# Suyashagarw/StreamOptima

Hardware: AMD Instinct MI355X
Metric: encoded Mpixels/sec at 1080p & 4K, 1/2/4/8 GPUs; PSNR delta vs reference (higher is better)
Workload: dtype u8

## Files before the change

### include/streamoptima.h

```cpp
#ifndef STREAMOPTIMA_H
#define STREAMOPTIMA_H

#include <stddef.h>
#include <stdint.h>

#ifdef __cplusplus
extern "C" {
#endif

#define SO_OK 0
#define SO_E_INVALID (-1)
#define SO_E_UNSUPPORTED (-2)
#define SO_MAX_REF 4
#define SO_ABI_VERSION 1

int so_abi_version(void);
const char* so_last_error(void);

int so_me_full_search(const uint8_t* cur, const uint8_t* const* refs, int nref, int H,
                      int W, int bs, int sr, int32_t* out_best, int32_t* out_sub,
                      void* stream);

int so_inter_tq_recon(const uint8_t* cur, const uint8_t* const* refs, int nref, int H,
                      int W, int bs, const int32_t* best, const int32_t* sub, int qp_rd,
// ... 17 lines not shown

#define SO_OPT_RUN_2PASS_FUSED 1
#define SO_OPT_FASTME_SERIAL 2
#define SO_OPT_FASTME_SEGMENT 3
#define SO_OPT_FASTME_WARMUP 4
#define SO_OPT_COUNT_SAD_OPS 5
#define SO_OPT_TEST_LOSE_FLAG 6
#define SO_OPT_RUN_ZERO_SKIP 7
#define SO_OPT_RUN_TALL_TILES 8
int so_set_option(int option, int value);
int so_get_option(int option);

#define SO_P_RUN_TIMEOUT_WORD 32
#define SO_P_RUN_FALLBACK_WORD 64
#define SO_P_RUN_SAD_OPS_WORD 66
#define SO_P_RUN_STALE_WORD 33
#define SO_P_RUN_GAP_WORD 34
#define SO_P_RUN_DIAG_WORD 96
#define SO_P_RUN_DIAG_MAGIC 0x534F0001u
size_t so_p_run_workspace_elems(int H, int W);
int so_p_run_resident_workgroups(int vbs);
int so_p_run_mode_resident_workgroups(int mode, int vbs);
int so_p_run_tile_rows(int H, int W, int conc);
int so_encode_p_run(const uint8_t* const* curs, int nframes, const uint8_t* ref0, int H, int W,
                    int bs, int sr, int qp_rd, const int32_t* qp_row, int vbs, double lam,
                    uint8_t* const* out_split,
                    int16_t* const* out_mv, int16_t* const* out_qtc, int32_t* const* out_tokens,
                    int32_t* const* out_mae_num, uint8_t* const* out_recon, int32_t* const* out_sse,
                    uint32_t* workspace, void* stream);

// ... 180 lines not shown
```

### streamoptima_amd/csrc/so_block.h

```cpp
#pragma once
#include "so_common.h"
#include "so_dct.h"

namespace so {

SO_DEV void wave_sync() {
    __builtin_amdgcn_fence(__ATOMIC_RELEASE, "wavefront");
    __builtin_amdgcn_wave_barrier();
    __builtin_amdgcn_fence(__ATOMIC_ACQUIRE, "wavefront");
}

SO_DEV int scan_index(int n, int i, int j) {
    const int k = i + j;
    const int before = (k < n) ? (k * (k + 1)) / 2 : n * n - ((2 * n - 1 - k) * (2 * n - k)) / 2;
    const int first_i = (k < n) ? 0 : k - n + 1;
    return before + (i - first_i);
}

template <int G>
SO_DEV int group_sum(int v) {
#pragma unroll
    for (int m = G / 2; m >= 1; m >>= 1) v += __shfl_xor(v, m, 64);
    return v;
}
// ... 162 lines not shown
#pragma unroll
    for (int r = 0; r < N; ++r) colp[r * P] = (uint32_t)__builtin_bit_cast(uint64_t, v[r]);
    wave_sync();
#pragma unroll
    for (int c = 0; c < N; ++c) lo[c] = rowp[c];
    wave_sync();
#pragma unroll
    for (int r = 0; r < N; ++r) colp[r * P] = (uint32_t)(__builtin_bit_cast(uint64_t, v[r]) >> 32);
    wave_sync();
#pragma unroll
    for (int c = 0; c < N; ++c)
        v[c] = __builtin_bit_cast(double, ((uint64_t)rowp[c] << 32) | (uint64_t)lo[c]);
    if constexpr (INVERSE) dct::dct3<N>(v, tw); else dct::dct2<N>(v, tw);
#pragma unroll
    for (int c = 0; c < N; ++c) out_row[c] = v[c];
    wave_sync();
}

template <class TWt>
SO_DEV void xform2d_fwd_i_half(double* lds, int l, const int* in_row, double* out_row, const TWt& tw) {
    constexpr int N = 16, PI = N + 1, P = 9;
    const int hl = l >> 3, cl = l & 7;
    double v[N];
    {
        int* const li = reinterpret_cast<int*>(lds);
#pragma unroll
        for (int c = 0; c < N; ++c) li[l * PI + c] = in_row[c];
        wave_sync();
        int x[N];
#pragma unroll
// ... 244 lines not shown
```

### streamoptima_amd/csrc/so_dct.h

```cpp
#pragma once
#include "so_common.h"

namespace so {
namespace dct {

constexpr double kTw16Dct[15] = {
    0x1.fd88da3d12526p-1, 0x1.f6297cff75cb0p-1, 0x1.e9f4156c62ddap-1, 0x1.d906bcf328d46p-1,
    0x1.c38b2f180bdb1p-1, 0x1.a9b66290ea1a3p-1, 0x1.8bc806b151741p-1, 0x1.6a09e667f3bccp-1,
    0x1.44cf325091dd6p-1, 0x1.1c73b39ae68c8p-1, 0x1.e2b5d3806f639p-2, 0x1.87de2a6aea961p-2,
    0x1.294062ed59f04p-2, 0x1.8f8b83c69a60ap-3, 0x1.917a6bc29b424p-4};
constexpr double kTw16Rf[9] = {
    0x1.d906bcf328d46p-1, 0x1.87de2a6aea963p-2, 0.0,
    0x1.6a09e667f3bccp-1, 0x1.6a09e667f3bcdp-1, 0.0,
    0x1.87de2a6aea963p-2, 0x1.d906bcf328d46p-1, 0.0};
constexpr double kSqrt2 = 0x1.6a09e667f3bcdp+0;
constexpr double kHsqt2 = 0x1.6a09e667f3bcdp-1;

struct TW16 {
    SO_DEV double dct(int i) const { return kTw16Dct[i]; }
    SO_DEV double hdct(int i) const { return 0.5 * kTw16Dct[i]; }
    SO_DEV double dct2x(int i) const { return 2 * kTw16Dct[i]; }
    SO_DEV double rf(int i) const { return kTw16Rf[i]; }
    SO_DEV double fct() const { return 0x1.6a09e667f3bcdp-3; }
    SO_DEV double sqrt2() const { return kSqrt2; }
// ... 15 lines not shown
    SO_DEV double hsqt2() const { return kHsqt2; }
};

#define SO_TW_D(i) kTw16Dct[i]
#define SO_TW_H(i) (0.5 * kTw16Dct[i])
static __constant__ double kTw16Tab[45] = {
    SO_TW_D(0), SO_TW_D(1), SO_TW_D(2), SO_TW_D(3), SO_TW_D(4), SO_TW_D(5), SO_TW_D(6), SO_TW_D(7),
    SO_TW_D(8), SO_TW_D(9), SO_TW_D(10), SO_TW_D(11), SO_TW_D(12), SO_TW_D(13), SO_TW_D(14),
    SO_TW_H(0), SO_TW_H(1), SO_TW_H(2), SO_TW_H(3), SO_TW_H(4), SO_TW_H(5), SO_TW_H(6), SO_TW_H(7),
    SO_TW_H(8), SO_TW_H(9), SO_TW_H(10), SO_TW_H(11), SO_TW_H(12), SO_TW_H(13), SO_TW_H(14),
    kTw16Rf[0], kTw16Rf[1], kTw16Rf[2], kTw16Rf[3], kTw16Rf[4], kTw16Rf[5], kTw16Rf[6], kTw16Rf[7], kTw16Rf[8],
    0x1.6a09e667f3bcdp-3, kSqrt2, kSqrt2 * 0.5, kHsqt2, 2 * kTw16Dct[7], 0.0};
#undef SO_TW_D
#undef SO_TW_H
typedef const __attribute__((address_space(4))) double* so_cdp;
struct TW16R {
    so_cdp p;
    SO_DEV double dct(int i) const { return p[i]; }
    SO_DEV double hdct(int i) const { return p[15 + i]; }
    SO_DEV double dct2x(int i) const { return i == 7 ? p[43] : 2 * p[i]; }
    SO_DEV double rf(int i) const { return p[30 + i]; }
    SO_DEV double fct() const { return p[39]; }
    SO_DEV double sqrt2() const { return p[40]; }
    SO_DEV double hsqrt2() const { return p[41]; }
    SO_DEV double hsqt2() const { return p[42]; }
};
SO_DEV TW16R tw16_table() {
    so_cdp q = (so_cdp)kTw16Tab;
    asm volatile("" : "+s"(q));
    return TW16R{q};
}
static __constant__ double kTw8Tab[21] = {
    kTw8Dct[0], kTw8Dct[1], kTw8Dct[2], kTw8Dct[3], kTw8Dct[4], kTw8Dct[5], kTw8Dct[6],
    0.5 * kTw8Dct[0], 0.5 * kTw8Dct[1], 0.5 * kTw8Dct[2], 0.5 * kTw8Dct[3], 0.5 * kTw8Dct[4],
    0.5 * kTw8Dct[5], 0.5 * kTw8Dct[6],
    kTw8Rf[0], kTw8Rf[1], 0x1.0p-2, kSqrt2, kSqrt2 * 0.5, kHsqt2, 2 * kTw8Dct[3]};
struct TW8R {
    so_cdp p;
    SO_DEV double dct(int i) const { return p[i]; }
    SO_DEV double hdct(int i) const { return p[7 + i]; }
    SO_DEV double dct2x(int i) const { return i == 3 ? p[20] : 2 * p[i]; }
    SO_DEV double rf(int i) const { return p[14 + i]; }
    SO_DEV double fct() const { return 0x1.0p-2; }
    SO_DEV double sqrt2() const { return p[17]; }
    SO_DEV double hsqrt2() const { return p[18]; }
    SO_DEV double hsqt2() const { return p[19]; }
};
SO_DEV TW8R tw8_table() {
    so_cdp q = (so_cdp)kTw8Tab;
    asm volatile("" : "+s"(q));
    return TW8R{q};
}

#define SO_PM(a, b, c, d) { a = (c) + (d); b = (c) - (d); }
#define SO_MULPM(a, b, c, d, e, f) { a = (c) * (e) + (d) * (f); b = (c) * (f) - (d) * (e); }

template <int IDO, int L1, class TW>
SO_DEV void radf2(const double* cc, double* ch, const TW& tw) {
#define CC(a, b, c) cc[(a) + IDO * ((b) + L1 * (c))]
#define CH(a, b, c) ch[(a) + IDO * ((b) + 2 * (c))]
#define WA(x, i) tw.rf((i) + (x) * (IDO - 1))
#pragma unroll
    for (int k = 0; k < L1; k++) SO_PM(CH(0, 0, k), CH(IDO - 1, 1, k), CC(0, k, 0), CC(0, k, 1));
    if constexpr ((IDO & 1) == 0) {
#pragma unroll
// ... 392 lines not shown
        c[kc] = tw.dct(k - 1) * t1 - tw.dct(kc - 1) * t2;
    }
    c[4] = (double)x[4] * tw.dct2x(3);
    Rfft<8>::forward(c, tw);
#pragma unroll
    for (int k = 1; k < 7; k += 2) {
        double t = c[k];
        c[k] -= c[k + 1];
        c[k + 1] += t;
    }
}

#undef SO_PM
#undef SO_MULPM

}
}
```

### streamoptima_amd/csrc/so_me.hip

```cpp
#include <stdlib.h>
#include <string.h>

#include <cstring>
#include <map>
#include <mutex>
#include <type_traits>
#include <utility>

#include "so_block.h"
#include "so_common.h"
#include "so_dpp.h"
#include "so_run.h"

namespace so {

SO_DEV uint64_t me_key(uint32_t sad, uint32_t l1, uint32_t ref, uint32_t scan) {
    return ((uint64_t)sad << 32) | ((uint64_t)l1 << 24) | ((uint64_t)ref << 16) | (uint64_t)scan;
}
constexpr uint64_t kNoKey = ~0ull;
constexpr uint32_t kDenseSadOps = 1152u * 256u;
#define SO_OPS_ADD(p, v) do { if (L.count_ops) atomicAdd((p), (v)); } while (0)

SO_DEV void decode_key(uint64_t k, int sr, int32_t* out) {
    if (k == kNoKey) {
// ... 513 lines not shown
extern "C" int so_debug_set_sea_stamps(void* p) {
    return (int)hipMemcpyToSymbol(HIP_SYMBOL(g_sea_stamps), &p, sizeof(p));
}
extern "C" int so_debug_set_run_stamps(void* p) {
    return (int)hipMemcpyToSymbol(HIP_SYMBOL(g_run_stamps), &p, sizeof(p));
}
#else
#define SO_STAMP_REC_SET(p) do { } while (0)
#define SO_SEA_STAMP(i, v) do { } while (0)
#endif

#define SO_MARK_NAMES(X) X(loop_top) X(stage_cur) X(stage_cur_int) X(stage_cur_edge) X(cur_sums) X(wait) \
    X(poll_iter) X(stage_win) X(stage_win_int) X(stage_win_edge) X(dense_tile) X(dense_tile_block) X(byte_sums) \
    X(block_top) X(bound) X(umin) X(umin_edge) X(ballots) X(bal_row) X(dense_fallback) X(survivors) X(sur_one) X(sur_le4) X(sur_pass) \
    X(search_end) X(decode_keys) X(tq_residual) X(tq_fwd) X(tq_quant) X(tq_tokens) X(tq_qtc_store) X(tq_inv) \
    X(tq_recon) X(tq_sse_records) X(post) X(done_flag) X(task_end) X(vbs_block) X(vbs_umin) X(vbs_list_a) \
    X(vbs_pass) X(vbs_list_b) X(vbs_final) X(vbs_dense) X(vbs_fwd) X(vbs_fwd_sub) X(vbs_final_q) X(vbs_inv) \
    X(vbs_inv_split) X(vbs_inv_end) X(wait_w0) X(keys_tail) X(p1_tq) X(p1_flag) X(p2_wait) X(p2_sums) X(p2_tq) \
    X(p2_flag)
#define SO_MARK_ENUM(n) kMark_##n,
enum SoMarkId { SO_MARK_NAMES(SO_MARK_ENUM) kMarkCount };
#undef SO_MARK_ENUM
#if defined(SO_MARKS_COUNT)
__device__ unsigned* g_mark_counts = nullptr;
__shared__ unsigned s_mark_cnt[64];
extern "C" int so_debug_set_mark_counts(void* p) {
    return (int)hipMemcpyToSymbol(HIP_SYMBOL(g_mark_counts), &p, sizeof(p));
}
SO_DEV void so_mark_hit(int id) {
    uint64_t sv, m;
    uint32_t f;
// ... 945 lines not shown
};

struct PHalo {
    uint8_t* up;
    uint8_t* dn;
    int up_end, dn_begin;
};

#ifdef SO_TQ_TW_LITERAL
#define SO_TQ_TW() dct::TW16{}
#define SO_TQ_TW8() dct::TW8{}
#else
#define SO_TQ_TW() dct::tw16_table()
#define SO_TQ_TW8() dct::tw8_table()
#endif
template <class G, bool SC1, bool HALO = false, bool TOK = false, bool HALFTQ = false, bool ZSKIP = false>
SO_DEV void tq16_exact(PTileLds<G, false, HALFTQ>& S, int g, int l, double* scratch, int bx0, int byt0, int nbx, int by0, int by1,
                       int W, int qp_rd, const int32_t* __restrict__ qp_row, const int32_t* __restrict__ qp_map,
                       const PFrameOut& o, const PHalo& hl = PHalo{}, bool qs = false) {
    constexpr int SR = G::SR, TBX = G::TBX;
    const int bxl = g % TBX, byl = g / TBX;
    const int gbx = bx0 + bxl, gby = byt0 + byl;
    if (gbx < nbx && gby < by1) {
        const size_t b = (size_t)(gby - by0) * nbx + gbx;
        const int x = gbx * 16, y = gby * 16;
        const int qpr = qp_map ? qp_map[(size_t)gby * nbx + gbx] : (qp_row ? qp_row[gby] : qp_rd);
        const int dx = S.mer[g][0], dy = S.mer[g][1], rf = S.mer[g][2], sad = S.mer[g][3];
        const int prow = byl * 16 + SR + dy + l, pcol = bxl * 16 + SR + dx;
        const uint32_t* crow = S.curt + (byl * 16 + l) * G::CPD + bxl * 4;
        double* dl = scratch;
        constexpr double kRne = 0x1.8p52;
        int q[16];
        if (qs) {
            const so_v4u* qr = reinterpret_cast<const so_v4u*>(reinterpret_cast<const int16_t*>(dl) + l * 16);
#pragma unroll
            for (int h = 0; h < 2; ++h) {
                const so_v4u v = qr[h];
#pragma unroll
                for (int e = 0; e < 4; ++e) {
                    q[8 * h + 2 * e] = (int)(int16_t)(v[e] & 0xFFFFu);
                    q[8 * h + 2 * e + 1] = (int)v[e] >> 16;
                }
            }
        } else {
            SO_MARK(tq_residual);
            int res[16];
            {
                uint32_t pw[4];
                win_row16<G::RP>(S.win, prow, pcol, pw);
#pragma unroll
                for (int k = 0; k < 4; ++k) {
                    const uint32_t cw = crow[k];
#pragma unroll
                    for (int e = 0; e < 4; ++e)
                        res[4 * k + e] = (int)((cw >> (8 * e)) & 255) - (int)((pw[k] >> (8 * e)) & 255);
                }
            }
            double tcr[16];
            SO_MARK(tq_fwd);
            static_assert(!HALFTQ || TOK, "the half scratch carries the forward transform only");
            if constexpr (HALFTQ)
                xform2d_fwd_i_half(dl, l, res, tcr, SO_TQ_TW());
            else if constexpr (G::TQDW)
                xform2d_rows_dw<false>(dl, l, res, tcr, SO_TQ_TW());
            else
                xform2d_rows<16, false>(dl, l, res, tcr, SO_TQ_TW());
            SO_MARK(tq_quant);
#pragma unroll
            for (int c = 0; c < 16; ++c)
                q[c] = (int)(uint32_t)__builtin_bit_cast(
                    uint64_t, __builtin_amdgcn_ldexp(__builtin_rint(tcr[c]), -q_exp_fast<16>(l, c, qpr)) + kRne);
        }
        SO_MARK(tq_tokens);
        const int tok = block_tokens<16>(nullptr, l, q);
        if constexpr (TOK) {
            if (l == 0) o.tokens[b] = tok;
            return;
        }
        SO_MARK(tq_qtc_store);
        store_row_i16<16>(o.qtc + b * 256 + l * 16, q);
        const auto finish = [&](const int (&rec)[16]) -> int {
            if constexpr (SC1) {
                so_v4u v;
#pragma unroll
                for (int k = 0; k < 4; ++k)
                    v[k] = (uint32_t)(rec[4 * k] & 255) | ((uint32_t)(rec[4 * k + 1] & 255) << 8) |
                           ((uint32_t)(rec[4 * k + 2] & 255) << 16) | ((uint32_t)(rec[4 * k + 3] & 255) << 24);
                uint8_t* rp = o.recon + (size_t)(y + l) * W + x;
// ... 21 lines not shown
                    crow2 = S.curt + ((g2 / TBX) * 16 + l2) * G::CPD + (g2 % TBX) * 4;
                }
#pragma unroll
                for (int k = 0; k < 4; ++k) {
                    const uint32_t cw = crow2[k];
#pragma unroll
                    for (int e = 0; e < 4; ++e) {
                        const int d = (int)((cw >> (8 * e)) & 255) - (rec[4 * k + e] & 255);
                        e2 += d * d;
                    }
                }
                e2 = group_sum<16>(e2);
            }
            return e2;
        };
        const auto full = [&]() -> int {
            int dq[16];
            double rd[16];
            dequant_row_int<16>(q, l, qpr, dq);
            SO_MARK(tq_inv);
            if constexpr (G::TQDW)
                xform2d_rows_dw<true>(dl, l, dq, rd, SO_TQ_TW());
            else
                xform2d_rows<16, true>(dl, l, dq, rd, SO_TQ_TW());
            SO_MARK(tq_recon);
            int rec[16];
            {
                uint32_t pw[4];
                win_row16<G::RP>(S.win, prow, pcol, pw);
#pragma unroll
                for (int c = 0; c < 16; ++c)
                    rec[c] = (int)((pw[c >> 2] >> (8 * (c & 3))) & 255) +
                             (int)(uint32_t)__builtin_bit_cast(uint64_t, rd[c] + kRne);
            }
            return finish(rec);
        };
        int sse;
        if constexpr (ZSKIP) {
            if (__builtin_amdgcn_ballot_w64(tok != 1) == 0) {
                int rec[16];
                uint32_t pw[4];
                win_row16<G::RP>(S.win, prow, pcol, pw);
#pragma unroll
                for (int c = 0; c < 16; ++c) rec[c] = (int)((pw[c >> 2] >> (8 * (c & 3))) & 255);
                sse = finish(rec);
            } else {
                sse = full();
            }
        } else {
            sse = full();
// ... 419 lines not shown
    SO_MARK(vbs_inv_end);
    if (o.sse) {
        sse = group_sum<16>(sse);
        if (l == 0) o.sse[b] = sse;
    }
}

SO_DEV void store_sc1_i16(int16_t* p, int v) {
    asm volatile("global_store_short %0, %1, off sc1" ::"v"(p), "v"(v) : "memory");
}
SO_DEV void store_sc1_i32(int32_t* p, int v) {
    asm volatile("global_store_dword %0, %1, off sc1" ::"v"(p), "v"(v) : "memory");
}

template <class G, bool SC1, class Pre = NoPre, bool HALO = false, bool TOK = false, bool VBS = false,
          class Post = NoPre, bool HALFTQ = false, bool ZSKIP = false, int LISTS = 0>
SO_DEV void ptile_body(PTileLds<G, VBS, HALFTQ>& S, int tile, const uint8_t* __restrict__ cur, const uint8_t* ref, int H, int W,
                       int by0, int by1, int qp_rd, const int32_t* __restrict__ qp_row,
                       const int32_t* __restrict__ qp_map, int32_t* __restrict__ out_best, const PFrameOut& o,
                       const Pre& pre = Pre(), const PHalo& hl = PHalo{}, double lam = 0.0,
                       const int* dense_flag = nullptr, int32_t* fb_out = nullptr, int count_ops = 0,
                       const Post& post = Post(), const int16_t* prev_mv = nullptr) {
    constexpr int SR = G::SR, TBX = G::TBX, TBY = G::TBY;
    using P = PTileGeo<G>;
    uint32_t* const b4w = reinterpret_cast<uint32_t*>(S.un);
    uint16_t* const list = reinterpret_cast<uint16_t*>(b4w + P::B4);
    constexpr int kUnDw = 2 * (VBS ? PTileGeoVbs<G>::U64 : PTileGeo<G, HALFTQ>::U64);
    int dense4 = 0;
#ifndef SO_DENSE_ONE
    if constexpr (3 * G::DCS + 32 <= kUnDw) {
        const int d = (int)((reinterpret_cast<uintptr_t>(b4w) - reinterpret_cast<uintptr_t>(S.win)) / 4);
// ... 54 lines not shown
        }
        if (SO_PROF_PHASE == 1 && ln < 16 * G::TQ_BPW && gq < G::NBLK) {
            const int bxl = gq % G::TBX, byl = gq / G::TBX, l = ln & 15;
            const int gbx = bx0 + bxl, gby = byt0 + byl;
            if (gbx < nbx && gby < by1) {
                const uint32_t* crow = S.curt + (byl * 16 + l) * G::CPD + bxl * 4;
                so_v4u v;
                for (int k = 0; k < 4; ++k) v[k] = crow[k];
                *reinterpret_cast<so_v4u*>(o.recon + (size_t)(gby * 16 + l) * W + gbx * 16) = v;
            }
        } else if (ln < 16 * G::TQ_BPW && gq < G::NBLK) {
            if constexpr (VBS)
                tq16_vbs_fwd<G, SC1, HALO>(S, gq, ln & 15, S.un + gq * kTqScratchVbs, bx0, byt0, nbx, by0, by1, W, qp_rd,
                                           qp_row, qp_map, lam, o);
            else
                tq16_exact<G, SC1, HALO, TOK, HALFTQ, ZSKIP>(S, gq, ln & 15, S.un + gq * tq_scratch<G, HALFTQ>(), bx0,
                                              byt0, nbx, by0, by1, W, qp_rd,
                                              qp_row, qp_map, o, hl, qs);
        }
    }
    if constexpr (VBS) {
        if (SO_PROF_PHASE != 1) {
            __syncthreads();
            const int ln = tid & 63, gq = (tid >> 6) * G::TQ_BPW + (ln >> 4);
            if (ln < 16 * G::TQ_BPW && gq < G::NBLK)
                tq16_vbs_inv<G, SC1, HALO>(S, gq, ln & 15, S.un, bx0, byt0, nbx, by0, by1, W, qp_rd,
                                           qp_row, qp_map, o, hl);
        }
    }
    SO_SEA_STAMP(7, __builtin_amdgcn_s_memtime());
    SO_MARK(post);
// ... 198 lines not shown

#ifndef SO_RUN_ACQUIRE
#define SO_RUN_ACQUIRE 1
#endif
#ifndef SO_RUN_ABORT_CHECK
#define SO_RUN_ABORT_CHECK 1
#endif
#ifndef SO_RUN_TIMEOUT_WORD
#define SO_RUN_TIMEOUT_WORD 32
#endif
#ifndef SO_RUN_DONE_BASE
#define SO_RUN_DONE_BASE 128
#endif
constexpr int kRunTimeoutWord = SO_RUN_TIMEOUT_WORD, kRunDoneBase = SO_RUN_DONE_BASE;
constexpr int kRunExitWord = 1, kRunEpochWord = 2, kRunFallbackWord = 64, kRunSadOpsWord = SO_P_RUN_SAD_OPS_WORD;
constexpr int kRunStaleWord = SO_P_RUN_STALE_WORD, kRunGapWord = SO_P_RUN_GAP_WORD, kRunClaimWord = 35;
constexpr int kRunDiagWord = SO_P_RUN_DIAG_WORD;
static_assert(kRunDoneBase >= kRunDiagWord + 32, "the diagnostic record precedes the done flags");
constexpr int kRunSingle = 0, kRunStripe = 1, kRunFPipe = 2, kRunTwoPass = 3, kRunFPipe2P = 4;
#ifdef SO_RUN_PROFILE
#define SO_RUN_PROF(word, cyc) \
    do { if (wave == 0) __hip_atomic_fetch_add(&ws[(word)], lane == 0 ? (uint32_t)((cyc) >> 10) : 0u, __ATOMIC_RELAXED, __HIP_MEMORY_SCOPE_AGENT); } while (0)
#else
#define SO_RUN_PROF(word, cyc) do { } while (0)
#endif

struct RunWait {
    int task, f, dep, tile, mode;
    uint32_t want, sys_want;
    unsigned long long limit;
// ... 143 lines not shown
    constexpr bool MERGE2P = MODE == kRunTwoPass;
    const int lag2 = ntiles - (tiles_x + 1);
    const int per_frame = TWOP && !MERGE2P ? 2 * ntiles : ntiles;
    const int ntasks = per_frame * nframes + (MERGE2P ? lag2 : 0);
    uint32_t* const done = ws + kRunDoneBase;
    uint32_t* const tilefb = ws + kRunDoneBase + 2 * (size_t)kRunMax * ntiles + (size_t)kRunMax * nbx * (H / 16);
    const int wave = __builtin_amdgcn_readfirstlane(tid >> 6);
    const int lane = tid & 63;
    const uint32_t one = lane == 0 ? 1u : 0u;
    __shared__ uint32_t s_fbsum;
    __shared__ unsigned long long s_ops;
    if (tid == 0) {
        s_fbsum = 0;
        s_ops = 0;
    }
#ifdef SO_MARKS_COUNT
    if (tid < 64) s_mark_cnt[tid] = 0u;
#endif
    const uint32_t ep0 = __builtin_amdgcn_readfirstlane(
        __hip_atomic_load(&ws[kRunEpochWord], __ATOMIC_RELAXED, __HIP_MEMORY_SCOPE_AGENT)) + 1u;
#ifndef SO_EP_REG
    __shared__ uint32_t s_ep;
    if (tid == 0) s_ep = ep0;
#define ep ((uint32_t)__builtin_amdgcn_readfirstlane(*(lds_vu32p)&s_ep))
#else
    const uint32_t ep = ep0;
#endif
    uint32_t nxt_v = 0;
    bool nxt_taken = false;
    for (;;) {
// ... 222 lines not shown
                nullptr, nullptr, count_ops, take_next, f > 0 ? a.out[f - 1].mv : nullptr);
            if (wave == 0) {
                __hip_atomic_store(done + (size_t)f * ntiles + tile, ep, __ATOMIC_RELAXED,
                                       __HIP_MEMORY_SCOPE_AGENT);
                if (lane == 0 && hl.up)
                    __hip_atomic_store(sp.peer_up_flags + (size_t)gf * tiles_x + tx, sp.epoch, __ATOMIC_RELAXED,
                                       __HIP_MEMORY_SCOPE_SYSTEM);
                if (lane == 1 && hl.dn)
                    __hip_atomic_store(sp.peer_dn_flags + (size_t)gf * tiles_x + tx, sp.epoch, __ATOMIC_RELAXED,
                                       __HIP_MEMORY_SCOPE_SYSTEM);
            }
        } else {
#ifdef SO_RUN_PROFILE
            const unsigned long long pt0 = __builtin_amdgcn_s_memtime();
#endif
            ptile_body<G, true, decltype(wait_ref), false, false, VBS, decltype(take_next), false, ZSKIP && !VBS, LISTS>(
                S, tile, a.cur[f], ref, H, W, 0, by1, qp_rd, qp_row, nullptr, nullptr, a.out[f], wait_ref, PHalo{}, lam,
                &s_dense, reinterpret_cast<int32_t*>(tilefb) + (size_t)f * ntiles + tile, count_ops, take_next,
                !VBS && dep >= 0 ? a.out[dep].mv : nullptr);
            SO_RUN_PROF(52, __builtin_amdgcn_s_memtime() - pt0);
            SO_MARK(done_flag);
            if (wave == 0 && !(HOOKS && task + 1 == sp.lose_task))
                __hip_atomic_store(done + (size_t)f * ntiles + tile, ep, __ATOMIC_RELAXED,
                                       __HIP_MEMORY_SCOPE_AGENT);
        }
        SO_MARK(task_end);
        if (pass == 1 && tid == 0) {
            s_fbsum += S.st[0];
            if constexpr (HOOKS) s_ops += S.st[2];
        }
#ifdef SO_STAMPS
// ... 4 lines not shown
            rec[11] = __builtin_amdgcn_s_memrealtime();
            rec[12] = ((unsigned long long)xcc << 32) | hw;
            rec[13] = __builtin_amdgcn_s_memtime();
        }
#endif
    }
#ifdef SO_MARKS_COUNT
    __syncthreads();
    if (tid < kMarkCount && g_mark_counts) atomicAdd(&g_mark_counts[tid], s_mark_cnt[tid]);
#endif
    if (wave == 0) {
        const uint32_t fbsum = __builtin_amdgcn_readfirstlane(s_fbsum);
        if (fbsum != 0u)
            __hip_atomic_fetch_add(&ws[kRunFallbackWord], lane == 0 ? fbsum : 0u, __ATOMIC_RELAXED,
                                   __HIP_MEMORY_SCOPE_AGENT);
        const unsigned long long ops = s_ops;
        if (ops != 0ull)
            __hip_atomic_fetch_add(reinterpret_cast<unsigned long long*>(ws + kRunSadOpsWord), lane == 0 ? ops : 0ull,
                                   __ATOMIC_RELAXED, __HIP_MEMORY_SCOPE_AGENT);
    }
    if (wave == 0) {
        const uint32_t o = __builtin_amdgcn_readfirstlane(
            __hip_atomic_fetch_add(&ws[kRunExitWord], one, __ATOMIC_RELAXED, __HIP_MEMORY_SCOPE_AGENT));
        if (o == gridDim.x - 1) {
            __hip_atomic_store(&ws[0], 0u, __ATOMIC_RELAXED, __HIP_MEMORY_SCOPE_AGENT);
            __hip_atomic_store(&ws[kRunExitWord], 0u, __ATOMIC_RELAXED, __HIP_MEMORY_SCOPE_AGENT);
            __hip_atomic_store(&ws[kRunEpochWord], ep, __ATOMIC_RELAXED, __HIP_MEMORY_SCOPE_AGENT);
        }
    }
}
// ... 506 lines not shown
```

### streamoptima_amd/engine.py

```python
from __future__ import annotations

import collections
import contextlib
from dataclasses import dataclass, field

import ctypes
import os

import torch

from . import _lib, runhealth

SLACK = 64
RUN_TIMEOUT_WORD = runhealth.TIMEOUT_WORD
RUN_FALLBACK_WORD = runhealth.FALLBACK_WORD


def alloc_planes(n: int, h: int, w: int, device, fill: int | None = None) -> torch.Tensor:
    flat = torch.empty(n * h * w + SLACK, dtype=torch.uint8, device=device)
    if fill is not None:
        flat.fill_(fill)
    else:
        flat[n * h * w:].zero_()
    return flat[: n * h * w].view(n, h, w)
# ... 357 lines not shown
            else:
                self.zero_skip = zero.item() >= self.ZERO_SKIP_SHARE * self.nb * len(outs)

    def take_sad_ops(self) -> int:
        ws = getattr(self, "_run_ws", None)
        return 0 if ws is None else runhealth.take_u64(ws, runhealth.SAD_OPS_WORD)

    def take_fallback_count(self) -> int:
        ws = getattr(self, "_run_ws", None)
        if ws is None:
            return 0
        n = int(ws[RUN_FALLBACK_WORD].item())
        ws[RUN_FALLBACK_WORD].zero_()
        return n

    def encode_i_rows(self, cur, by0: int, by1: int, qp_rd: int, out: FrameSymbols,
                      qp_row_dev: torch.Tensor | None = None, qp_map_dev: torch.Tensor | None = None,
                      qp_row=None) -> FrameSymbols:
        self._check_plane(cur, "cur")
        rc = self.lib.so_encode_i_rows_ex(
            cur.data_ptr(), self.h, self.w, self.bs, self.sr, int(by0), int(by1), int(qp_rd), _lib.ptr(qp_row_dev),
            _lib.ptr(qp_map_dev), int(self.vbs), self.lam, out.split.data_ptr(), out.mv.data_ptr(),
            out.qtc.data_ptr(), out.tokens.data_ptr(), out.mae_num.data_ptr(), out.recon.data_ptr(),
            _lib.ptr(out.sse), self.scratch.data_ptr(), _lib.stream_handle(self.device))
        _lib.check(rc, "so_encode_i_rows_ex")
        out.frame_type, out.qp_rd = 0, int(qp_rd)
        out.qp_row = None if qp_row is None else list(qp_row)
        return out

    def recon_inter(self, refs: list, split, mv, qtc, qp: int, qp_row=None, out=None,
# ... 161 lines not shown
```

### streamoptima_amd/runhealth.py

```python
from __future__ import annotations

import torch

TIMEOUT_WORD = 32
STALE_WORD = 33
GAP_WORD = 34
CLAIM_WORD = 35
FALLBACK_WORD = 64
SAD_OPS_WORD = 66
DIAG_WORD = 96
DIAG_MAGIC = 0x534F0001
TICK_US = 0.01

MODES = {0: "one GPU", 1: "stripe", 2: "frame pipeline", 3: "two-pass", 4: "frame pipeline, two-pass"}
FIELDS = ("magic", "task", "frame", "dep", "tile", "epoch", "gop_epoch", "mode", "lanes_waited",
          "lanes_remote", "poll_ticks", "wall_ticks", "descheduled_ticks", "_13", "arrival_ticks", "hw_id",
          "xcc_id", "block", "grid", "lanes_set_by_atomic_read")


def decode_record(words) -> dict | None:
    w = [int(x) & 0xFFFFFFFF for x in words]
    if w[0] != DIAG_MAGIC:
        return None
    rec = {k: w[i] for i, k in enumerate(FIELDS) if not k.startswith("_") and k != "magic"}
# ... 86 lines not shown
```

Measured before the change: 170,800.

## Add fast 16-point DCT path with certified rounding and exact fallback

Adds a faster 16-point forward/inverse DCT (scaled DCT-IV decomposition with fused multiply-adds and constants in SGPR) for the single-mode plain P-run transform-quant. After quantization, coefficients whose values lie near a rounding boundary are checked; if the fast result could differ from the exact one, the block is recomputed with the exact transform. The inverse path does the same using a fixed-point margin test. Fallback counts are accumulated into new workspace words. The intent is fewer FLOPs in the transform stage, at the cost of extra ballots, register pressure and occasional recomputation.

```diff
diff --git a/include/streamoptima.h b/include/streamoptima.h
--- a/include/streamoptima.h
+++ b/include/streamoptima.h
@@ -55,6 +55,7 @@
 #define SO_P_RUN_TIMEOUT_WORD 32
 #define SO_P_RUN_FALLBACK_WORD 64
 #define SO_P_RUN_SAD_OPS_WORD 66
+#define SO_P_RUN_TQ_FALLBACK_WORD 68
 #define SO_P_RUN_STALE_WORD 33
 #define SO_P_RUN_GAP_WORD 34
 #define SO_P_RUN_DIAG_WORD 96
diff --git a/streamoptima_amd/csrc/so_block.h b/streamoptima_amd/csrc/so_block.h
--- a/streamoptima_amd/csrc/so_block.h
+++ b/streamoptima_amd/csrc/so_block.h
@@ -200,6 +200,53 @@
     if constexpr (INVERSE) dct::dct3<N>(v, tw); else dct::dct2<N>(v, tw);
 #pragma unroll
     for (int c = 0; c < N; ++c) out_row[c] = v[c];
+    wave_sync();
+}
+
+template <bool INVERSE, bool DW, class FT>
+SO_DEV void xform2d_fast(double* lds, int l, const int* in_row, double (&v)[16], const FT& ft) {
+    constexpr int N = 16, P = N + 1;
+    typedef __attribute__((address_space(3))) uint32_t* lds_u32p;
+    lds_u32p rowp = (lds_u32p)(reinterpret_cast<uint32_t*>(lds) + l * P);
+    lds_u32p colp = (lds_u32p)(reinterpret_cast<uint32_t*>(lds) + l);
+    if constexpr (DW) asm volatile("" : "+v"(rowp), "+v"(colp));
+    {
+#pragma unroll
+        for (int c = 0; c < N; ++c) rowp[c] = (uint32_t)in_row[c];
+        wave_sync();
+        int x[N];
+#pragma unroll
+        for (int r = 0; r < N; ++r) x[r] = (int)colp[r * P];
+        wave_sync();
+        if constexpr (INVERSE) {
+#pragma unroll
+            for (int r = 0; r < N; ++r) v[r] = (double)x[r];
+            dct::dct3_16_fast(v, ft);
+        } else {
+            dct::dct2_16_fast_i(x, v, ft);
+        }
+    }
+    if constexpr (DW) {
+        uint32_t lo[N];
+#pragma unroll
+        for (int r = 0; r < N; ++r) colp[r * P] = (uint32_t)__builtin_bit_cast(uint64_t, v[r]);
+        wave_sync();
+#pragma unroll
+        for (int c = 0; c < N; ++c) lo[c] = rowp[c];
+        wave_sync();
+#pragma unroll
+        for (int r = 0; r < N; ++r) colp[r * P] = (uint32_t)(__builtin_bit_cast(uint64_t, v[r]) >> 32);
+        wave_sync();
+#pragma unroll
+        for (int c = 0; c < N; ++c) v[c] = __builtin_bit_cast(double, ((uint64_t)rowp[c] << 32) | (uint64_t)lo[c]);
+    } else {
+#pragma unroll
+        for (int r = 0; r < N; ++r) lds[r * P + l] = v[r];
+        wave_sync();
+#pragma unroll
+        for (int c = 0; c < N; ++c) v[c] = lds[l * P + c];
+    }
+    if constexpr (INVERSE) dct::dct3_16_fast(v, ft); else dct::dct2_16_fast(v, ft);
     wave_sync();
 }
 
diff --git a/streamoptima_amd/csrc/so_dct.h b/streamoptima_amd/csrc/so_dct.h
--- a/streamoptima_amd/csrc/so_dct.h
+++ b/streamoptima_amd/csrc/so_dct.h
@@ -53,6 +53,11 @@
 #undef SO_TW_D
 #undef SO_TW_H
 typedef const __attribute__((address_space(4))) double* so_cdp;
+#if defined(__HIP_DEVICE_COMPILE__)
+#define SO_SGPR_BARRIER(q) asm volatile("" : "+s"(q))
+#else
+#define SO_SGPR_BARRIER(q) (void)(q)
+#endif
 struct TW16R {
     so_cdp p;
     SO_DEV double dct(int i) const { return p[i]; }
@@ -66,7 +71,7 @@
 };
 SO_DEV TW16R tw16_table() {
     so_cdp q = (so_cdp)kTw16Tab;
-    asm volatile("" : "+s"(q));
+    SO_SGPR_BARRIER(q);
     return TW16R{q};
 }
 static __constant__ double kTw8Tab[21] = {
@@ -87,7 +92,7 @@
 };
 SO_DEV TW8R tw8_table() {
     so_cdp q = (so_cdp)kTw8Tab;
-    asm volatile("" : "+s"(q));
+    SO_SGPR_BARRIER(q);
     return TW8R{q};
 }
 
@@ -510,5 +515,149 @@
 #undef SO_PM
 #undef SO_MULPM
 
-}
-}
+constexpr double kFastBoundFwd = 2.33e-10, kPocketBoundFwd = 4.14e-11;
+constexpr double kFastBoundInv = 2.57e-9, kPocketBoundInv = 1.66e-9;
+constexpr double kFastDeltaFwd = 0x1.0p-30, kFastDeltaInv = 0x1.8p-24;
+static_assert(kFastDeltaFwd >= kFastBoundFwd + kPocketBoundFwd && kFastDeltaInv >= kFastBoundInv + kPocketBoundInv,
+              "a flag threshold below the sum of the two error bounds");
+
+#define SO_FAST16_CONSTANTS                                                                        \
+    0x1.0000000000000p-2, 0x1.4e7ae9144f0fcp-2, 0x1.1517a7bdb3895p-3, 0x1.63150b15e8536p-2,        \
+    0x1.2d062ef88e319p-2, 0x1.92469c0dcf32dp-3, 0x1.1a855dec071b5p-4, 0x1.684b9c80f1a8bp-2,        \
+    0x1.5a730c6c21c67p-2, 0x1.3f4a237187eafp-2, 0x1.17dc13dab2dd6p-2, 0x1.cb598cc4beea0p-3,        \
+    0x1.5553e3f5b5e58p-3, 0x1.a4608aafa8527p-4, 0x1.1be35182fe5aap-5, 0x1.6a09e667f3bcdp+0,        \
+    0x1.d906bcf328d46p+0, 0x1.87de2a6aea963p-1, 0x1.f6297cff75cb0p+0, 0x1.a9b66290ea1a3p+0,        \
+    0x1.1c73b39ae68c8p+0, 0x1.8f8b83c69a60bp-2
+constexpr double kFast16[22] = {SO_FAST16_CONSTANTS};
+static __constant__ double kFast16Tab[22] = {SO_FAST16_CONSTANTS};
+#undef SO_FAST16_CONSTANTS
+struct FT16 {
+    SO_DEV double k(int i) const { return kFast16[i]; }
+};
+struct FT16R {
+    so_cdp p;
+    SO_DEV double k(int i) const { return p[i]; }
+};
+SO_DEV FT16R ft16_table() {
+    so_cdp q = (so_cdp)kFast16Tab;
+    SO_SGPR_BARRIER(q);
+    return FT16R{q};
+}
+
+template <class FT>
+SO_DEV double fast_c16(const FT& t, int base, int q) {
+    q &= 31;
+    if (q > 16) q = 32 - q;
+    const bool neg = q > 8;
+    if (neg) q = 16 - q;
+    const double c = t.k(base + (q - 1) / 2);
+    return neg ? -c : c;
+}
+
+template <class FT>
+SO_DEV void dct4_8_fast(const double (&b)[8], double (&y)[8], const FT& t) {
+    double u[8], ap[4], bp[4];
+#pragma unroll
+    for (int n = 0; n < 8; ++n) u[n] = b[n] * t.k(7 + n);
+#pragma unroll
+    for (int i = 0; i < 4; ++i) {
+        ap[i] = u[i] + u[7 - i];
+        bp[i] = u[i] - u[7 - i];
+    }
+    const double e0 = ap[0] + ap[3], e1 = ap[1] + ap[2], f0 = ap[0] - ap[3], f1 = ap[1] - ap[2];
+    y[0] = e0 + e1;
+#pragma unroll
+    for (int j = 0; j < 4; ++j) {
+        double acc = -y[2 * j];
+#pragma unroll
+        for (int i = 0; i < 4; ++i) acc = __builtin_fma(fast_c16(t, 18, (2 * i + 1) * (2 * j + 1)), bp[i], acc);
+        y[2 * j + 1] = acc;
+        if (j == 0) y[2] = __builtin_fma(t.k(17), f1, __builtin_fma(t.k(16), f0, -acc));
+        if (j == 1) y[4] = __builtin_fma(t.k(15), e0 - e1, -acc);
+        if (j == 2) y[6] = __builtin_fma(-t.k(16), f1, __builtin_fma(t.k(17), f0, -acc));
+    }
+}
+
+template <class FT>
+SO_DEV void dct2_16_fast_tail(double e0pe1, double e0me1, double f0, double f1, const double (&d)[4],
+                              const double (&b)[8], double (&c)[16], const FT& t) {
+    c[0] = e0pe1 * t.k(0);
+    c[8] = e0me1 * t.k(0);
+    c[4] = __builtin_fma(t.k(2), f1, t.k(1) * f0);
+    c[12] = __builtin_fma(-t.k(1), f1, t.k(2) * f0);
+#pragma unroll
+    for (int j = 0; j < 4; ++j) {
+        double acc = fast_c16(t, 3, 2 * j + 1) * d[0];
+#pragma unroll
+        for (int i = 1; i < 4; ++i) acc = __builtin_fma(fast_c16(t, 3, (2 * i + 1) * (2 * j + 1)), d[i], acc);
+        c[4 * j + 2] = acc;
+    }
+    double y[8];
+    dct4_8_fast(b, y, t);
+#pragma unroll
+    for (int j = 0; j < 8; ++j) c[2 * j + 1] = y[j];
+}
+
+template <class FT = FT16>
+SO_DEV void dct2_16_fast(double (&c)[16], const FT& t = FT{}) {
+    double a[8], b[8], cc[4], d[4];
+#pragma unroll
+    for (int i = 0; i < 8; ++i) {
+        a[i] = c[i] + c[15 - i];
+        b[i] = c[i] - c[15 - i];
+    }
+#pragma unroll
+    for (int i = 0; i < 4; ++i) {
+        cc[i] = a[i] + a[7 - i];
+        d[i] = a[i] - a[7 - i];
+    }
+    const double e0 = cc[0] + cc[3], e1 = cc[1] + cc[2];
+    dct2_16_fast_tail(e0 + e1, e0 - e1, cc[0] - cc[3], cc[1] - cc[2], d, b, c, t);
+}
+
+template <class FT = FT16>
+SO_DEV void dct2_16_fast_i(const int (&x)[16], double (&c)[16], const FT& t = FT{}) {
+    int a[8], cc[4];
+    double b[8], d[4];
+#pragma unroll
+    for (int i = 0; i < 8; ++i) {
+        a[i] = x[i] + x[15 - i];
+        b[i] = (double)(x[i] - x[15 - i]);
+    }
+#pragma unroll
+    for (int i = 0; i < 4; ++i) {
+        cc[i] = a[i] + a[7 - i];
+        d[i] = (double)(a[i] - a[7 - i]);
+    }
+    const int e0 = cc[0] + cc[3], e1 = cc[1] + cc[2];
+    dct2_16_fast_tail((double)(e0 + e1), (double)(e0 - e1), (double)(cc[0] - cc[3]), (double)(cc[1] - cc[2]), d, b,
+                      c, t);
+}
+
+template <class FT = FT16>
+SO_DEV void dct3_16_fast(double (&c)[16], const FT& t = FT{}) {
+    const double p = t.k(0) * c[0];
+    const double e0 = __builtin_fma(t.k(0), c[8], p), e1 = __builtin_fma(-t.k(0), c[8], p);
+    const double f0 = __builtin_fma(t.k(2), c[12], t.k(1) * c[4]), f1 = __builtin_fma(-t.k(1), c[12], t.k(2) * c[4]);
+    const double cc[4] = {e0 + f0, e1 + f1, e1 - f1, e0 - f0};
+    double a[8], xo[8], bo[8];
+#pragma unroll
+    for (int i = 0; i < 4; ++i) {
+        double acc = fast_c16(t, 3, 2 * i + 1) * c[2];
+#pragma unroll
+        for (int j = 1; j < 4; ++j) acc = __builtin_fma(fast_c16(t, 3, (2 * i + 1) * (2 * j + 1)), c[4 * j + 2], acc);
+        a[i] = cc[i] + acc;
+        a[7 - i] = cc[i] - acc;
+    }
+#pragma unroll
+    for (int j = 0; j < 8; ++j) xo[j] = c[2 * j + 1];
+    dct4_8_fast(xo, bo, t);
+#pragma unroll
+    for (int i = 0; i < 8; ++i) {
+        c[i] = a[i] + bo[i];
+        c[15 - i] = a[i] - bo[i];
+    }
+}
+
+}
+}
diff --git a/streamoptima_amd/csrc/so_me.hip b/streamoptima_amd/csrc/so_me.hip
--- a/streamoptima_amd/csrc/so_me.hip
+++ b/streamoptima_amd/csrc/so_me.hip
@@ -551,7 +551,7 @@
     X(poll_iter) X(stage_win) X(stage_win_int) X(stage_win_edge) X(dense_tile) X(dense_tile_block) X(byte_sums) \
     X(block_top) X(bound) X(umin) X(umin_edge) X(ballots) X(bal_row) X(dense_fallback) X(survivors) X(sur_one) X(sur_le4) X(sur_pass) \
     X(search_end) X(decode_keys) X(tq_residual) X(tq_fwd) X(tq_quant) X(tq_tokens) X(tq_qtc_store) X(tq_inv) \
-    X(tq_recon) X(tq_sse_records) X(post) X(done_flag) X(task_end) X(vbs_block) X(vbs_umin) X(vbs_list_a) \
+    X(tq_recon) X(tq_fwd_near) X(tq_fwd_fallback) X(tq_inv_fallback) X(tq_sse_records) X(post) X(done_flag) X(task_end) X(vbs_block) X(vbs_umin) X(vbs_list_a) \
     X(vbs_pass) X(vbs_list_b) X(vbs_final) X(vbs_dense) X(vbs_fwd) X(vbs_fwd_sub) X(vbs_final_q) X(vbs_inv) \
     X(vbs_inv_split) X(vbs_inv_end) X(wait_w0) X(keys_tail) X(p1_tq) X(p1_flag) X(p2_wait) X(p2_sums) X(p2_tq) \
     X(p2_flag)
@@ -1527,7 +1527,12 @@
 #define SO_TQ_TW() dct::tw16_table()
 #define SO_TQ_TW8() dct::tw8_table()
 #endif
-template <class G, bool SC1, bool HALO = false, bool TOK = false, bool HALFTQ = false, bool ZSKIP = false>
+#ifndef SO_TQ_FAST
+#define SO_TQ_FAST 1
+#endif
+#define SO_TQ_FT() dct::ft16_table()
+template <class G, bool SC1, bool HALO = false, bool TOK = false, bool HALFTQ = false, bool ZSKIP = false,
+          bool FAST = false>
 SO_DEV void tq16_exact(PTileLds<G, false, HALFTQ>& S, int g, int l, double* scratch, int bx0, int byt0, int nbx, int by0, int by1,
                        int W, int qp_rd, const int32_t* __restrict__ qp_row, const int32_t* __restrict__ qp_map,
                        const PFrameOut& o, const PHalo& hl = PHalo{}, bool qs = false) {
@@ -1535,14 +1540,33 @@
     const int bxl = g % TBX, byl = g / TBX;
     const int gbx = bx0 + bxl, gby = byt0 + byl;
     if (gbx < nbx && gby < by1) {
-        const size_t b = (size_t)(gby - by0) * nbx + gbx;
-        const int x = gbx * 16, y = gby * 16;
+        size_t b = (size_t)(gby - by0) * nbx + gbx;
+        int x = gbx * 16, y = gby * 16;
         const int qpr = qp_map ? qp_map[(size_t)gby * nbx + gbx] : (qp_row ? qp_row[gby] : qp_rd);
         const int dx = S.mer[g][0], dy = S.mer[g][1], rf = S.mer[g][2], sad = S.mer[g][3];
         const int prow = byl * 16 + SR + dy + l, pcol = bxl * 16 + SR + dx;
         const uint32_t* crow = S.curt + (byl * 16 + l) * G::CPD + bxl * 4;
         double* dl = scratch;
         constexpr double kRne = 0x1.8p52;
+        const auto derive = [&]() {
+            if constexpr (FAST) {
+                asm volatile("" : "+v"(g), "+v"(l));
+                const int gbx2 = bx0 + g % TBX, gby2 = byt0 + g / TBX;
+                b = (size_t)(gby2 - by0) * nbx + gbx2;
+                x = gbx2 * 16;
+                y = gby2 * 16;
+                dl = S.un + g * tq_scratch<G, HALFTQ>();
+            }
+        };
+        const auto rows_of = [&](int g2, int l2, int& prow2, int& pcol2, const uint32_t*& crow2) {
+            asm volatile("" : "+v"(g2), "+v"(l2));
+            const int bxl2 = g2 % TBX, byl2 = g2 / TBX;
+            lds_vu32p mp = (lds_vu32p)reinterpret_cast<const uint32_t*>(&S.mer[g2]);
+            const uint32_t w0 = mp[0];
+            prow2 = byl2 * 16 + SR + ((int)w0 >> 16) + l2;
+            pcol2 = bxl2 * 16 + SR + (int)(int16_t)(w0 & 0xFFFFu);
+            crow2 = S.curt + (byl2 * 16 + l2) * G::CPD + bxl2 * 4;
+        };
         int q[16];
         if (qs) {
             const so_v4u* qr = reinterpret_cast<const so_v4u*>(reinterpret_cast<const int16_t*>(dl) + l * 16);
@@ -1558,20 +1582,85 @@
         } else {
             SO_MARK(tq_residual);
             int res[16];
-            {
+            const auto load_res = [&](int prow_, int pcol_, const uint32_t* crow_) {
                 uint32_t pw[4];
-                win_row16<G::RP>(S.win, prow, pcol, pw);
+                win_row16<G::RP>(S.win, prow_, pcol_, pw);
 #pragma unroll
                 for (int k = 0; k < 4; ++k) {
-                    const uint32_t cw = crow[k];
+                    const uint32_t cw = crow_[k];
 #pragma unroll
                     for (int e = 0; e < 4; ++e)
                         res[4 * k + e] = (int)((cw >> (8 * e)) & 255) - (int)((pw[k] >> (8 * e)) & 255);
                 }
-            }
+            };
+            load_res(prow, pcol, crow);
             double tcr[16];
             SO_MARK(tq_fwd);
             static_assert(!HALFTQ || TOK, "the half scratch carries the forward transform only");
+            static_assert(!FAST || (!HALFTQ && !TOK && !HALO), "the fast transforms: the plain run only");
+            const int sc_hi2 = (1023 - 2 - qpr) << 20;
+            const auto quant_fma = [&](bool certify) -> bool {
+                int sc_hi = (1023 - qpr - (l == 15 ? 1 : 0)) << 20;
+                bool flag = false;
+#pragma unroll
+                for (int c0 = 0; c0 < 16; c0 += 4) {
+                    uint64_t nm[4], any = 0;
+#pragma unroll
+                    for (int j = 0; j < 4; ++j) {
+                        const int c = c0 + j;
+                        const double sc = __builtin_bit_cast(double, (uint64_t)(uint32_t)sc_hi << 32);
+                        const double r = __builtin_rint(tcr[c]);
+                        q[c] = (int)(uint32_t)__builtin_bit_cast(uint64_t, __builtin_fma(r, sc, kRne));
+                        if (certify) {
+                            nm[j] = __builtin_amdgcn_ballot_w64(__builtin_fabs(tcr[c] - r) >= 0.5 - dct::kFastDeltaFwd);
+                            any |= nm[j];
+                        }
+                        if (c < 15) sc_hi = __builtin_amdgcn_update_dpp(sc_hi2, sc_hi, 0x101, 0xF, 0xF, false);
+                    }
+#ifdef SO_TQ_CENSUS_NO_NEAR
+                    any = 0;
+#endif
+                    if (certify && any != 0) {
+                        SO_MARK(tq_fwd_near);
+#pragma unroll
+                        for (int j = 0; j < 4; ++j) {
+                            if (nm[j] != 0) {
+                                const int c = c0 + j;
+                                const double sc = __builtin_bit_cast(
+                                    double, (uint64_t)(uint32_t)((1023 - q_exp_fast<16>(l, c, qpr)) << 20) << 32);
+                                const double r = __builtin_rint(tcr[c]), d = tcr[c] - r;
+                                const double r2 = r + __builtin_copysign(1.0, d);
+                                const int q2 = (int)(uint32_t)__builtin_bit_cast(uint64_t, __builtin_fma(r2, sc, kRne));
+                                flag |= __builtin_fabs(d) >= 0.5 - dct::kFastDeltaFwd && q2 != q[c];
+                            }
+                        }
+                        SO_MARK(tq_quant);
+                    }
+                }
+                return certify && __builtin_amdgcn_ballot_w64(flag) != 0;
+            };
+            if constexpr (FAST) {
+                xform2d_fast<false, G::TQDW>(dl, l, res, tcr, SO_TQ_FT());
+                asm volatile("" : "+v"(tcr[0]), "+v"(tcr[1]), "+v"(tcr[2]), "+v"(tcr[3]), "+v"(tcr[4]), "+v"(tcr[5]),
+                             "+v"(tcr[6]), "+v"(tcr[7]));
+                asm volatile("" : "+v"(tcr[8]), "+v"(tcr[9]), "+v"(tcr[10]), "+v"(tcr[11]), "+v"(tcr[12]), "+v"(tcr[13]),
+                             "+v"(tcr[14]), "+v"(tcr[15]));
+                SO_MARK(tq_quant);
+                if (quant_fma(true)) {
+                    SO_MARK(tq_fwd_fallback);
+                    const uint64_t act = __builtin_amdgcn_ballot_w64(true);
+                    if ((int)(threadIdx.x & 63) == __builtin_ctzll(act)) atomicAdd(reinterpret_cast<uint32_t*>(&S.msum[0]), 1u);
+                    int prow2, pcol2;
+                    const uint32_t* crow2;
+                    rows_of(g, l, prow2, pcol2, crow2);
+                    load_res(prow2, pcol2, crow2);
+                    if constexpr (G::TQDW)
+                        xform2d_rows_dw<false>(dl, l, res, tcr, SO_TQ_TW());
+                    else
+                        xform2d_rows<16, false>(dl, l, res, tcr, SO_TQ_TW());
+                    quant_fma(false);
+                }
+            } else {
             if constexpr (HALFTQ)
                 xform2d_fwd_i_half(dl, l, res, tcr, SO_TQ_TW());
             else if constexpr (G::TQDW)
@@ -1583,8 +1672,10 @@
             for (int c = 0; c < 16; ++c)
                 q[c] = (int)(uint32_t)__builtin_bit_cast(
                     uint64_t, __builtin_amdgcn_ldexp(__builtin_rint(tcr[c]), -q_exp_fast<16>(l, c, qpr)) + kRne);
+            }
         }
         SO_MARK(tq_tokens);
+        derive();
         const int tok = block_tokens<16>(nullptr, l, q);
         if constexpr (TOK) {
             if (l == 0) o.tokens[b] = tok;
@@ -1636,26 +1727,81 @@
             }
             return e2;
         };
-        const auto full = [&]() -> int {
+        const auto full_exact = [&](const int (&ql)[16]) -> int {
             int dq[16];
             double rd[16];
-            dequant_row_int<16>(q, l, qpr, dq);
-            SO_MARK(tq_inv);
+            dequant_row_int<16>(ql, l, qpr, dq);
+            if constexpr (!FAST) SO_MARK(tq_inv);
             if constexpr (G::TQDW)
                 xform2d_rows_dw<true>(dl, l, dq, rd, SO_TQ_TW());
             else
                 xform2d_rows<16, true>(dl, l, dq, rd, SO_TQ_TW());
-            SO_MARK(tq_recon);
+            if constexpr (!FAST) SO_MARK(tq_recon);
+            derive();
             int rec[16];
             {
+                int prow2 = prow, pcol2 = pcol;
+                if constexpr (FAST) {
+                    const uint32_t* crow2;
+                    rows_of(g, l, prow2, pcol2, crow2);
+                }
                 uint32_t pw[4];
-                win_row16<G::RP>(S.win, prow, pcol, pw);
+                win_row16<G::RP>(S.win, prow2, pcol2, pw);
 #pragma unroll
                 for (int c = 0; c < 16; ++c)
                     rec[c] = (int)((pw[c >> 2] >> (8 * (c & 3))) & 255) +
                              (int)(uint32_t)__builtin_bit_cast(uint64_t, rd[c] + kRne);
             }
             return finish(rec);
+        };
+        const auto full = [&]() -> int {
+            if constexpr (FAST) {
+                {
+                    int dq[16], rec[16];
+                    double rd[16];
+                    {
+                        int k = qpr + (l == 15 ? 1 : 0);
+#pragma unroll
+                        for (int c = 0; c < 16; ++c) {
+                            dq[c] = (int)((uint32_t)q[c] << k);
+                            if (c < 15) k = __builtin_amdgcn_update_dpp(qpr + 2, k, 0x101, 0xF, 0xF, false);
+                        }
+                    }
+                    SO_MARK(tq_inv);
+                    xform2d_fast<true, G::TQDW>(dl, l, dq, rd, SO_TQ_FT());
+                    asm volatile("" : "+v"(rd[0]), "+v"(rd[1]), "+v"(rd[2]), "+v"(rd[3]), "+v"(rd[4]), "+v"(rd[5]),
+                                 "+v"(rd[6]), "+v"(rd[7]));
+                    asm volatile("" : "+v"(rd[8]), "+v"(rd[9]), "+v"(rd[10]), "+v"(rd[11]), "+v"(rd[12]), "+v"(rd[13]),
+                                 "+v"(rd[14]), "+v"(rd[15]));
+                    SO_MARK(tq_recon);
+                    derive();
+                    constexpr double kFix = 0x1.8p28 + 0.5;
+                    uint32_t mn = 0xFFFFFFFFu;
+                    {
+                        int prow2, pcol2;
+                        const uint32_t* crow2;
+                        rows_of(g, l, prow2, pcol2, crow2);
+                        uint32_t pw[4];
+                        win_row16<G::RP>(S.win, prow2, pcol2, pw);
+#pragma unroll
+                        for (int c = 0; c < 16; ++c) {
+                            const uint32_t gfix = (uint32_t)__builtin_bit_cast(uint64_t, rd[c] + kFix);
+                            rec[c] = (int)(((((pw[c >> 2] >> (8 * (c & 3))) & 255u) << 24) + gfix) >> 24);
+                            const uint32_t t = (gfix + 2u) << 8;
+                            mn = t < mn ? t : mn;
+                        }
+                    }
+                    if (__builtin_amdgcn_ballot_w64(mn <= (4u << 8)) == 0) return finish(rec);
+                }
+                SO_MARK(tq_inv_fallback);
+                const uint64_t act = __builtin_amdgcn_ballot_w64(true);
+                if ((int)(threadIdx.x & 63) == __builtin_ctzll(act)) atomicAdd(reinterpret_cast<uint32_t*>(&S.msum[1]), 1u);
+                int qf[16];
+                load_row_i16<16>(o.qtc + b * 256 + l * 16, qf);
+                return full_exact(qf);
+            } else {
+                return full_exact(q);
+            }
         };
         int sse;
         if constexpr (ZSKIP) {
@@ -2105,7 +2251,7 @@
 }
 
 template <class G, bool SC1, class Pre = NoPre, bool HALO = false, bool TOK = false, bool VBS = false,
-          class Post = NoPre, bool HALFTQ = false, bool ZSKIP = false, int LISTS = 0>
+          class Post = NoPre, bool HALFTQ = false, bool ZSKIP = false, int LISTS = 0, bool FASTTQ = false>
 SO_DEV void ptile_body(PTileLds<G, VBS, HALFTQ>& S, int tile, const uint8_t* __restrict__ cur, const uint8_t* ref, int H, int W,
                        int by0, int by1, int qp_rd, const int32_t* __restrict__ qp_row,
                        const int32_t* __restrict__ qp_map, int32_t* __restrict__ out_best, const PFrameOut& o,
@@ -2190,7 +2336,7 @@
                 tq16_vbs_fwd<G, SC1, HALO>(S, gq, ln & 15, S.un + gq * kTqScratchVbs, bx0, byt0, nbx, by0, by1, W, qp_rd,
                                            qp_row, qp_map, lam, o);
             else
-                tq16_exact<G, SC1, HALO, TOK, HALFTQ, ZSKIP>(S, gq, ln & 15, S.un + gq * tq_scratch<G, HALFTQ>(), bx0,
+                tq16_exact<G, SC1, HALO, TOK, HALFTQ, ZSKIP, FASTTQ>(S, gq, ln & 15, S.un + gq * tq_scratch<G, HALFTQ>(), bx0,
                                               byt0, nbx, by0, by1, W, qp_rd,
                                               qp_row, qp_map, o, hl, qs);
         }
@@ -2419,6 +2565,7 @@
 #endif
 constexpr int kRunTimeoutWord = SO_RUN_TIMEOUT_WORD, kRunDoneBase = SO_RUN_DONE_BASE;
 constexpr int kRunExitWord = 1, kRunEpochWord = 2, kRunFallbackWord = 64, kRunSadOpsWord = SO_P_RUN_SAD_OPS_WORD;
+constexpr int kRunTqFallbackWord = SO_P_RUN_TQ_FALLBACK_WORD;
 constexpr int kRunStaleWord = SO_P_RUN_STALE_WORD, kRunGapWord = SO_P_RUN_GAP_WORD, kRunClaimWord = 35;
 constexpr int kRunDiagWord = SO_P_RUN_DIAG_WORD;
 static_assert(kRunDoneBase >= kRunDiagWord + 32, "the diagnostic record precedes the done flags");
@@ -2592,6 +2739,10 @@
         s_fbsum = 0;
         s_ops = 0;
     }
+    constexpr bool kFastTq = SO_TQ_FAST != 0 && MODE == kRunSingle && !VBS && G::TBY == 3;
+    if constexpr (kFastTq) {
+        if (tid < 2) S.msum[tid] = 0;
+    }
 #ifdef SO_MARKS_COUNT
     if (tid < 64) s_mark_cnt[tid] = 0u;
 #endif
@@ -2844,7 +2995,7 @@
 #ifdef SO_RUN_PROFILE
             const unsigned long long pt0 = __builtin_amdgcn_s_memtime();
 #endif
-            ptile_body<G, true, decltype(wait_ref), false, false, VBS, decltype(take_next), false, ZSKIP && !VBS, LISTS>(
+            ptile_body<G, true, decltype(wait_ref), false, false, VBS, decltype(take_next), false, ZSKIP && !VBS, LISTS, kFastTq>(
                 S, tile, a.cur[f], ref, H, W, 0, by1, qp_rd, qp_row, nullptr, nullptr, a.out[f], wait_ref, PHalo{}, lam,
                 &s_dense, reinterpret_cast<int32_t*>(tilefb) + (size_t)f * ntiles + tile, count_ops, take_next,
                 !VBS && dep >= 0 ? a.out[dep].mv : nullptr);
@@ -2879,6 +3030,15 @@
         if (fbsum != 0u)
             __hip_atomic_fetch_add(&ws[kRunFallbackWord], lane == 0 ? fbsum : 0u, __ATOMIC_RELAXED,
                                    __HIP_MEMORY_SCOPE_AGENT);
+        if constexpr (kFastTq) {
+#pragma unroll
+            for (int d = 0; d < 2; ++d) {
+                const uint32_t n = __builtin_amdgcn_readfirstlane((uint32_t)S.msum[d]);
+                if (n != 0u)
+                    __hip_atomic_fetch_add(&ws[kRunTqFallbackWord + d], lane == 0 ? n : 0u, __ATOMIC_RELAXED,
+                                           __HIP_MEMORY_SCOPE_AGENT);
+            }
+        }
         const unsigned long long ops = s_ops;
         if (ops != 0ull)
             __hip_atomic_fetch_add(reinterpret_cast<unsigned long long*>(ws + kRunSadOpsWord), lane == 0 ? ops : 0ull,
diff --git a/streamoptima_amd/engine.py b/streamoptima_amd/engine.py
--- a/streamoptima_amd/engine.py
+++ b/streamoptima_amd/engine.py
@@ -395,6 +395,15 @@
         ws[RUN_FALLBACK_WORD].zero_()
         return n
 
+    def take_tq_fallback_counts(self) -> tuple:
+        ws = getattr(self, "_run_ws", None)
+        if ws is None:
+            return 0, 0
+        w = ws[runhealth.TQ_FALLBACK_WORD:runhealth.TQ_FALLBACK_WORD + 2]
+        n = tuple(int(v) & 0xFFFFFFFF for v in w.cpu().tolist())
+        w.zero_()
+        return n
+
     def encode_i_rows(self, cur, by0: int, by1: int, qp_rd: int, out: FrameSymbols,
                       qp_row_dev: torch.Tensor | None = None, qp_map_dev: torch.Tensor | None = None,
                       qp_row=None) -> FrameSymbols:
diff --git a/streamoptima_amd/runhealth.py b/streamoptima_amd/runhealth.py
--- a/streamoptima_amd/runhealth.py
+++ b/streamoptima_amd/runhealth.py
@@ -8,6 +8,7 @@
 CLAIM_WORD = 35
 FALLBACK_WORD = 64
 SAD_OPS_WORD = 66
+TQ_FALLBACK_WORD = 68
 DIAG_WORD = 96
 DIAG_MAGIC = 0x534F0001
 TICK_US = 0.01
```

Measured after the change: 179,200, median of 6. 1.05x the previous value.
